# EmbodiedVision/emfusion

Hardware: AMD Instinct MI355X
Metric: frames/sec (integrate+raycast+EM-assoc) (higher is better)
Workload: dtype f32

## Files before the change

emfusion_amd/_lib.py:

```python
from __future__ import annotations

import ctypes as C
import os
import re
from pathlib import Path

PKG_DIR = Path(__file__).resolve().parent
REPO_ROOT = PKG_DIR.parent
LIB_PATH = PKG_DIR / "libemf_hip.so"
HEADER_PATH = REPO_ROOT / "include" / "emf_hip.h"

EMF_OK = 0


class EmfImage(C.Structure):

    _fields_ = [("data", C.c_void_p), ("pitch", C.c_size_t), ("width", C.c_int32),
                ("height", C.c_int32)]


class EmfHipError(RuntimeError):
    def __init__(self, fn: str, code: int, msg: str):
        super().__init__(f"{fn} failed with {code}: {msg}")
        self.code = code
# ... 102 lines not shown
    "emf_hip_trackPrepare": [_FP, _FP, C.c_int, C.c_float, _STREAM],
    "emf_hip_trackIterate": [_FP, _FP, C.c_int, _IMG, C.c_void_p, _FP, C.c_size_t,
                             C.c_int, _STREAM],
    "emf_hip_trackStep": [_FP, _FP, C.c_int, _IMG, C.c_void_p, _FP, C.c_size_t,
                          C.c_int, C.c_int, C.c_void_p, C.c_uint32, C.c_void_p, _STREAM],
    "emf_hip_trackWeightImages": [_FP, _FP, C.c_int, _IMG, C.c_void_p, _FP, C.c_size_t, _FP, _FP, _STREAM],
    "emf_hip_computePoseGradients": [_FP, _FP, _IMG, _F9, _F9, _I3, C.c_float, _FP, _STREAM],
    "emf_hip_integrateBatched": [_FP, _FP, _I3, C.c_int, _FP, _IMG, _IMG, _F9, C.c_int, _FP,
                                 _STREAM],
    "emf_hip_integrateCullScratchBytes": [_I3, C.c_int],
    "emf_hip_integrateBatchedCulled": [_FP, _FP, _I3, C.c_int, _FP, _IMG, _IMG, _F9, _FP, C.c_uint32, _FP, _FP,
                                       _STREAM],
    "emf_hip_integrateDirtyMapBytes": [_I3],
    "emf_hip_integrateBatchedCulledOut": [_FP, _FP, _I3, C.c_int, _FP, _IMG, _IMG, _F9, C.c_void_p, C.c_int, _FP,
                                          C.c_uint32, _FP, _FP, _STREAM],
    "emf_hip_integratePrepareOut": [C.c_void_p, _I3, C.c_int, _FP, _STREAM],
    "emf_hip_visibilityFlags": [_FP, C.c_int, C.c_int, _FP, _FP, _STREAM],
    "emf_hip_resetBrickFlags": [_FP, _I3, _STREAM],
    "emf_hip_packHitKeys": [C.c_int, _I3, _IMG, _IMG, _FP, C.c_int, C.c_int, _STREAM],
    "emf_hip_compositeFromKeys": [_FP, C.c_int, _I3, C.c_int, _I3, _IMG, _IMG, _IMG, _IMG, _IMG,
                                  _IMG, _IMG, _IMG, _IMG, _IMG, _IMG, _IMG, _IMG, C.c_int, _FP,
                                  _STREAM],
    "emf_hip_visibilityFlagsIndexed": [_FP, C.c_int, _I3, C.c_int, _FP, _STREAM],
}


class EmfVolumeOut(C.Structure):
    _fields_ = [("tsdf", C.c_void_p), ("weights", C.c_void_p), ("dirtyPrev", C.c_void_p), ("dirtyNext", C.c_void_p)]


# ... 68 lines not shown
    return _lib


def _bind(lib: C.CDLL) -> C.CDLL:
    for name, argtypes in SIGNATURES.items():
        fn = getattr(lib, name)
        fn.argtypes = argtypes
        fn.restype = C.c_int
    lib.emf_hip_trackScratchBytes.restype = C.c_size_t
    lib.emf_hip_unseenTileBytes.restype = C.c_size_t
    lib.emf_hip_pointStatsScratchBytes.restype = C.c_size_t
    lib.emf_hip_meshScratchBytes.restype = C.c_size_t
    lib.emf_hip_meshScratchBytesBatched.restype = C.c_size_t
    lib.emf_hip_integrateCullScratchBytes.restype = C.c_size_t
    lib.emf_hip_integrateDirtyMapBytes.restype = C.c_size_t
    lib.emf_hip_signMapBytes.restype = C.c_size_t
    lib.emf_hip_raycastFarBoundBytes.restype = C.c_size_t
    lib.emf_hip_relevantTileBytes.restype = C.c_size_t
    lib.emf_hip_peerBufferBytes.restype = C.c_size_t
    lib.emf_hip_peerRaycastSlotBytes.restype = C.c_size_t
    lib.emf_hip_maskAssociationMassBytes.restype = C.c_size_t
    lib.emf_hip_maskAssociationMassScratchBytes.restype = C.c_size_t
    lib.emf_hip_last_error_string.argtypes = []
    lib.emf_hip_last_error_string.restype = C.c_char_p
    return lib


def check(fn_name: str, rc: int) -> None:
    if rc != EMF_OK:
        msg = load().emf_hip_last_error_string().decode(errors="replace")
# ... 2 lines not shown
```

emfusion_amd/csrc/batched.hip:

```cpp
#include <cstdlib>

#include "march_wave.hpp"
#include "peer_core.hpp"

namespace emf_hip {
namespace {

struct PoseTable {
    emf_pose_t p[EMF_MAX_BATCH];
};

__device__ __forceinline__ M33 pose_R(const emf_pose_t& p) {
    return M33{{p.R[0], p.R[1], p.R[2]}, {p.R[3], p.R[4], p.R[5]}, {p.R[6], p.R[7], p.R[8]}};
}
__device__ __forceinline__ V3 pose_t(const emf_pose_t& p) { return V3{p.t[0], p.t[1], p.t[2]}; }


#ifndef EMF_ESTEP_PIXELS
#define EMF_ESTEP_PIXELS 64
#define EMF_ESTEP_LANES 4
#endif
constexpr int kEstepPixels = EMF_ESTEP_PIXELS;
constexpr int kEstepLanes = EMF_ESTEP_LANES;

// ... 720 lines not shown
struct IntegrateOutTable {
    float* tsdf[EMF_MAX_BATCH];
    float* weights[EMF_MAX_BATCH];
    const uint8_t* dirtyPrev[EMF_MAX_BATCH];
    uint8_t* dirtyNext[EMF_MAX_BATCH];
};

struct IntegrateCullArgs {
    IntegrateBatchArgs b;
    int boxStart[EMF_MAX_BATCH + 1];
    unsigned* list;
    unsigned* count;
    IntegrateOutTable out;
    int haveOut;
    int deepTiles;
};


__device__ __forceinline__ IntegrateGeom geom_of(const IntegrateBatchArgs& a, int m) {
    const emf_model_t& md = a.models[m];
    IntegrateGeom g;
    g.depth = a.depth;
    g.invLambda = a.invLambda;
    g.assoc = Img<const float>{md.assoc, static_cast<size_t>(a.w) * sizeof(float)};
    g.w = a.w;
    g.h = a.h;
    g.R = pose_R(a.poses.p[m]);
    g.t = pose_t(a.poses.p[m]);
    g.K = a.K;
    g.pinhole = a.pinhole;
// ... 4 lines not shown
    return g;
}

__global__ __launch_bounds__(256) void k_integrate_cull(const IntegrateCullArgs a) {
    const int i = blockIdx.x * 256 + threadIdx.x;
    {
        float mx = 0.f;
        const int npix = a.b.w * a.b.h, stride = gridDim.x * 256;
        for (int p = i; p < npix; p += stride) {
            const float d = a.b.depth.row(p / a.b.w)[p % a.b.w];
            mx = d > mx ? d : mx;
        }
#pragma unroll
        for (int o = 32; o > 0; o >>= 1) mx = fmaxf(mx, __shfl_xor(mx, o));
        if ((threadIdx.x & 63) == 0 && mx > 0.f) atomicMax(a.count + 1, __float_as_uint(mx));
    }
    bool keep = false;
    unsigned entry = 0;
    if (i < a.boxStart[a.b.nmodels]) {
        int m = 0;
        while (m + 1 < a.b.nmodels && i >= a.boxStart[m + 1]) ++m;
        const bool open = !a.b.visible || a.b.visible[m] != 0;
        if (open || a.haveOut) {
            const IntegrateGeom g = geom_of(a.b, m);
            const int box = i - a.boxStart[m];
            if (open && a.b.stats && box == 0)
                atomicAdd(a.b.stats, static_cast<unsigned long long>(g.n.x) * g.n.y * g.n.z);
            const int nbx = (g.n.x + kBoxX - 1) / kBoxX, nby = (g.n.y + kBoxY - 1) / kBoxY;
            const int bx = box % nbx, by = (box / nbx) % nby, bz = box / (nbx * nby);
            const int x0 = bx * kBoxX, y0 = by * kBoxY, z0 = bz * kBoxZ;
// ... 27 lines not shown
            }
            entry = (static_cast<unsigned>(m) << 24) | static_cast<unsigned>(box);
        }
    }
    const unsigned long long mask = __ballot(keep);
    if (mask == 0ull) return;
    const int lane = threadIdx.x & 63;
    unsigned base = 0;
    if (lane == __ffsll(static_cast<long long>(mask)) - 1) base = atomicAdd(a.count, static_cast<unsigned>(__popcll(mask)));
    base = __shfl(base, __ffsll(static_cast<long long>(mask)) - 1);
    if (keep) a.list[base + __popcll(mask & ((1ull << lane) - 1ull))] = entry;
}

template <bool OUT>
__device__ __forceinline__ void integrate_listed_tile(const IntegrateCullArgs& a, unsigned e, unsigned sub,
                                                      unsigned* lds) {
    const unsigned entry = a.list[e];
    const int m = static_cast<int>(entry >> 24), box = static_cast<int>(entry & 0xffffffu);
    IntegrateGeom g = geom_of(a.b, m);
    g.maxDepthBits = a.deepTiles ? a.count + 1 : nullptr;
    const emf_model_t& md = a.b.models[m];
    const int nbx = (g.n.x + kBoxX - 1) / kBoxX, nby = (g.n.y + kBoxY - 1) / kBoxY;
    const int bx = box % nbx, by = (box / nbx) % nby, bz = box / (nbx * nby);
    const int dx = static_cast<int>(sub % EMF_INT_BOX_X), dy = static_cast<int>((sub / EMF_INT_BOX_X) % EMF_INT_BOX_Y),
              dz = static_cast<int>(sub / (EMF_INT_BOX_X * EMF_INT_BOX_Y));
    const int x0 = (EMF_INT_BOX_X * bx + dx) * kTileX, y0 = (EMF_INT_BOX_Y * by + dy) * kTileY,
              z0 = (EMF_INT_BOX_Z * bz + dz) * kTileZ;
    if (x0 < g.n.x && y0 < g.n.y && z0 < g.n.z) {
        const size_t t = tile_index(g.n, x0, y0, z0), nt = tile_count(g.n);
        uint8_t* sp = md.signMaps ? md.signMaps + t : nullptr;
        if constexpr (OUT) {
            const uint8_t* dp = a.out.dirtyPrev[m];
            const int force = (dp[t] ? 1 : 0) | (dp[nt + t] ? 2 : 0);
            integrate_tile<true>(g, md.tsdf, md.weights, nullptr, x0, y0, z0, lds, a.out.tsdf[m],
                                 a.out.weights[m], force, a.out.dirtyNext[m] + t, a.out.dirtyNext[m] + nt + t,
                                 a.b.visible && a.b.visible[m] == 0, sp, sp ? sp + nt : nullptr,
                                 md.unseenTiles ? md.unseenTiles + t : nullptr);
        } else {
            integrate_tile(g, md.tsdf, md.weights, nullptr, x0, y0, z0, lds, nullptr, nullptr, 0, nullptr, nullptr,
                           false, sp, sp ? sp + nt : nullptr, md.unseenTiles ? md.unseenTiles + t : nullptr);
        }
    }
}

template <bool OUT>
__attribute__((amdgpu_waves_per_eu(EMF_INT_WPE, EMF_INT_WPE)))
__global__ __launch_bounds__(256) void k_integrate_listed(const IntegrateCullArgs a) {
    __shared__ unsigned lds[32];
    const unsigned e = blockIdx.x / kBoxTiles;
    if (e >= *a.count) return;
    integrate_listed_tile<OUT>(a, e, blockIdx.x % kBoxTiles, lds);
}

template <bool OUT>
__global__ __launch_bounds__(256) void k_integrate_listed_rest(const IntegrateCullArgs a, unsigned first) {
    __shared__ unsigned lds[32];
    const unsigned todo = *a.count;
    for (unsigned e = first + blockIdx.x / kBoxTiles; e < todo; e += gridDim.x / kBoxTiles) {
        integrate_listed_tile<OUT>(a, e, blockIdx.x % kBoxTiles, lds);
        __syncthreads();
    }
}

struct DilateBatchArgs {
    const emf_model_t* models;
    int nmodels;
    int brickStart[EMF_MAX_BATCH + 1];
    const int32_t* visible;
};

__global__ __launch_bounds__(256) void k_dilate_batched(const DilateBatchArgs a) {
    const int i = blockIdx.x * 256 + threadIdx.x;
    if (i >= a.brickStart[a.nmodels]) return;
    int m = 0;
// ... 456 lines not shown
    EMF_REQUIRE_PTR(scratch_dev);
    if (nmodels < 1 || nmodels > EMF_MAX_BATCH) return fail(EMF_E_LIMIT, "integratePrepareOut: nmodels = %d", nmodels);
    hipError_t e = hipMemsetAsync(scratch_dev, 0, 2 * sizeof(unsigned), as_stream(stream));
    for (int m = 0; e == hipSuccess && out_host && m < nmodels; ++m) {
        if (!out_host[m].dirtyNext) return fail(EMF_E_NULL, "integratePrepareOut: model %d has no dirtyNext map", m);
        EMF_TRY(check_res(res_host + 3 * m));
        e = hipMemsetAsync(out_host[m].dirtyNext, 0, emf_hip_integrateDirtyMapBytes(res_host + 3 * m), as_stream(stream));
    }
    if (e != hipSuccess) {
        set_error("integratePrepareOut: memset: %s", hipGetErrorString(e));
        return static_cast<int>(e);
    }
    return EMF_OK;
}

int emf_hip_integrateBatchedCulledOut(const emf_model_t* models_dev, const emf_pose_t* poseOC_host,
                                      const int32_t* res_host, int nmodels, const int32_t* visible_dev,
                                      const emf_image_t* depth, const emf_image_t* invLambda,
                                      const float K[9], const emf_volume_out_t* out_host, int prepared,
                                      void* scratch_dev, uint32_t launchBoxes, uint32_t* survivors_out_dev,
                                      uint64_t* stats, emf_stream_t stream) {
    EMF_TRY(check_batch(models_dev, poseOC_host, nmodels, "integrateBatchedCulled"));
    EMF_REQUIRE_PTR(res_host);
    EMF_REQUIRE_PTR(scratch_dev);
    EMF_TRY(check_image(depth, 4, "integrateBatchedCulled: depth"));
    if (invLambda) {
        EMF_TRY(check_image(invLambda, 4, "integrateBatchedCulled: invLambda"));
        EMF_TRY(check_same_size(depth, invLambda, "depth", "invLambda"));
    }
    EMF_REQUIRE_PTR(K);
    IntegrateCullArgs a;
    a.b.models = models_dev;
    a.b.nmodels = nmodels;
    a.boxStart[0] = 0;
    for (int m = 0; m < nmodels; ++m) {
        const int32_t* r = res_host + 3 * m;
// ... 10 lines not shown
    a.b.visible = visible_dev;
    a.b.stats = reinterpret_cast<unsigned long long*>(stats);
    a.b.depth = img<const float>(depth);
    a.b.invLambda = invLambda ? img<const float>(invLambda) : Img<const float>{nullptr, 0};
    a.b.w = depth->width;
    a.b.h = depth->height;
    a.b.K = m33_from(K);
    a.b.pinhole = is_pinhole(a.b.K);
    a.count = static_cast<unsigned*>(scratch_dev);
    a.list = a.count + 4;
    a.out = IntegrateOutTable{};
    a.haveOut = out_host ? 1 : 0;
    const char* dt = std::getenv("EMF_DEEP_TILES");
    const bool deepTiles = !(dt && dt[0] == '0');
    a.deepTiles = deepTiles ? 1 : 0;
    const unsigned total = static_cast<unsigned>(a.boxStart[nmodels]);
    const hipError_t e = prepared ? hipSuccess : hipMemsetAsync(a.count, 0, 2 * sizeof(unsigned), as_stream(stream));
    if (e != hipSuccess) {
        set_error("integrateBatchedCulled: memset: %s", hipGetErrorString(e));
        return static_cast<int>(e);
    }
    if (out_host) {
        for (int m = 0; m < nmodels; ++m) {
            const emf_volume_out_t& o = out_host[m];
            if (!o.tsdf || !o.weights || !o.dirtyPrev || !o.dirtyNext)
                return fail(EMF_E_NULL, "integrateBatchedCulledOut: model %d: tsdf / weights / dirtyPrev / dirtyNext "
                            "of the second copy are all required", m);
            a.out.tsdf[m] = o.tsdf;
            a.out.weights[m] = o.weights;
            a.out.dirtyPrev[m] = o.dirtyPrev;
// ... 45 lines not shown
```

emfusion_amd/csrc/core/EMFusion.cpp:

```cpp
#include "EMFusion.hpp"
#include "EMFusionDetail.hpp"
#include "Readers.hpp"

#include <algorithm>
#include <chrono>
#include <cmath>
#include <cstdio>
#include <cstdlib>
#include <cstring>

namespace emf {

using namespace detail;

EMFusion::EMFusion(const Params& _params, TSDF::Gradients gradients,
                   std::shared_ptr<Communicator> _comm)
    : params(_params),
      gradMode(gradients),
      comm(std::move(_comm)),
      background(_params.globalVolumeDims, _params.globalVoxelSize,
                 _params.globalRelTruncDist * _params.globalVoxelSize, _params.volumePose,
                 _params.tsdfParams, _params.frameSize, gradients),
      depthFiltered(_params.frameSize),
      invLambda(_params.frameSize),
// ... 24 lines not shown
    }
    ignorePerson = params.ignore_person;
    const char* env = std::getenv("EMF_PER_VOLUME");
    forceLegacy = env && env[0] == '1';
    const char* bb = std::getenv("EMF_BG_BANDS");
    bgBands = !(bb && bb[0] == '0');
    const char* ic = std::getenv("EMF_INT_CULL");
    cullBoxes = !(ic && ic[0] == '0');
    const char* oc = debugEnv("EMF_OBJ_CULL");
    objCull = oc && oc[0] == '1';
    if (const char* tc = debugEnv("EMF_TRACK_CHUNK")) trackChunk = std::atoi(tc);
    if (const char* tw = debugEnv("EMF_TRACK_WINDOW")) trackWindow = std::atoi(tw);
    if (const char* fp = debugEnv("EMF_FUSE_POINTS")) fusePoints = fp[0] != '0';
    if (const char* fv = debugEnv("EMF_FUSE_VISIBILITY")) fuseVisibility = fv[0] != '0';
    if (const char* ef = debugEnv("EMF_EARLY_FAR_BOUNDS")) earlyFarBounds = ef[0] != '0';
    const char* bo = std::getenv("EMF_BG_OVERLAP");
    bgOverlap = !(bo && bo[0] == '0');
    const char* fb = std::getenv("EMF_FAR_BOUNDS");
    useFarBounds = !(fb && fb[0] == '0');
    const char* rf = debugEnv("EMF_RAY_FOOTPRINTS");
    useFootprints = !(rf && rf[0] == '0');
    if (const char* mr = std::getenv("EMF_MARCH_ROWS")) {
        marchLanes = std::atoi(mr);
        if (marchLanes != 1 && marchLanes != 2 && marchLanes != 4)
            throw HipError(std::string("EMFusion: EMF_MARCH_ROWS=") + mr + " (1, 2 or 4 lanes per background ray)", EMF_E_ARG);
    }
    const char* au = std::getenv("EMF_ASYNC_UPLOAD");
    asyncUpload = !(au && au[0] == '0');
    const char* lt = std::getenv("EMF_LAMBDA_TABLE");
    useLambdaTable = !(lt && lt[0] == '0');
// ... 191 lines not shown
        tiled &= md.res[0] % 4 == 0;
    }
    integrateCullScratch = DeviceBuffer();
    if (cullBoxes && tiled && TSDF::brickFlagMode() == 0)
        integrateCullScratch = DeviceBuffer(emf_hip_integrateCullScratchBytes(
            resHost.data(), std::min(static_cast<int>(modelsHost.size()), EMF_MAX_BATCH)));
    batched = !forceLegacy && gradMode == TSDF::Gradients::OnTheFly;
    farBounds = DeviceBuffer();
    if (batched && useFarBounds)
        farBounds = DeviceBuffer(2 * emf_hip_raycastFarBoundBytes(static_cast<int>(modelsHost.size()),
                                                                  params.frameSize.width, params.frameSize.height));
    if (batched && !integrateCullScratch.empty() && bgOverlap && bgCullScratch.empty()) {
        background.enableDoubleBuffer();
        bgCullScratch = DeviceBuffer(emf_hip_integrateCullScratchBytes(resHost.data(), 1));
    }
    tableSel = 0;
    hipCheck(hipMemcpy(modelTable.data(), modelsHost.data(),
                       modelsHost.size() * sizeof(emf_model_t), hipMemcpyHostToDevice),
             "model table upload");
    if (batched) {
        if (background.doubleBuffered()) {
            std::vector<emf_model_t> alt = modelsHost;
            const emf_volume_out_t back = background.backBuffers();
            alt[0].tsdf = back.tsdf;
            alt[0].weights = back.weights;
            hipCheck(hipMemcpy(modelTable.as<emf_model_t>() + EMF_MAX_MODELS, alt.data(),
                               alt.size() * sizeof(emf_model_t), hipMemcpyHostToDevice),
                     "model table upload");
        }
        std::vector<int32_t> vis(modelsHost.size(), 0);
// ... 424 lines not shown
void EMFusion::integrateBackgroundAsync() {
    if (!overlapUsable() || bgInFlight) return;
    if (bgBackStale) {
        quiesce();
        background.resyncBack();
        bgBackStale = false;
        bgPrepared = false;
    }
    aux.waitFor(main);
    const emf_pose_t oc = toPose(pose.inv() * background.getPose());
    const double vox = static_cast<double>(resHost[0]) * resHost[1] * resHost[2];
    const emf_image_t il = invLambda.view();
    const emf_volume_out_t out = background.backBuffers();
    {
        auto kt = ktimers.scope(KernelTimers::IntegrateBg, vox, aux);
        emfCheck(emf_hip_integrateBatchedCulledOut(currentTable(), &oc, resHost.data(), 1, nullptr, &depth,
                                                   useLambdaTable ? &il : nullptr, params.intr.val, &out,
                                                   bgPrepared ? 1 : 0, bgCullScratch.data(), 0, nullptr,
                                                   integrateStatsDev.as<uint64_t>(), aux.abi()),
                 "integrateBatchedCulledOut");
    }
    aux.record();
    emf_volume_out_t next = out;
    next.dirtyNext = const_cast<uint8_t*>(out.dirtyPrev);
    emfCheck(emf_hip_integratePrepareOut(&next, resHost.data(), 1, bgCullScratch.data(), aux.abi()),
             "integratePrepareOut");
    bgPrepared = true;
    bgInFlight = true;
    bgListPending = true;
    forkFrame = frameCount;
}

void EMFusion::joinBackground() {
    if (!bgInFlight) return;
    rebuildBackgroundList();
// ... 116 lines not shown
```

emfusion_amd/csrc/core/EMFusion.hpp:

```cpp
#pragma once

#include <algorithm>
#include <list>
#include <map>
#include <string>
#include <memory>
#include <set>
#include <vector>

#include "Communicator.hpp"
#include "KernelTimers.hpp"
#include "ObjTSDF.hpp"
#include "Output.hpp"
#include "TSDF.hpp"

namespace emf {

struct RGBD {
    Size size;
    const float* depth = nullptr;
    const uint8_t* rgb = nullptr;
};

struct FrameInputs {
// ... 320 lines not shown
    DeviceBuffer farBounds;
    int farSel = 0;
    float* farBoundsHalf() const { return farBounds.as<float>() + static_cast<size_t>(farSel) * (farBounds.bytes() / 2 / sizeof(float)); }
    int forkFrame = -2;
    bool farBoundsReady = false;
    bool earlyFarBounds = true;
    bool peerFused = false;
    int bandRowsPending = 0;
    Stream lists{streamPriority("EMF_PRIO_LISTS", -1)};
    bool bgListPending = false;
    bool bgPrepared = false;
    void rebuildBackgroundList();
    void computeFarBounds(const std::vector<emf_pose_t>& co);
    void joinFarBounds();
    DeviceBuffer bgCullScratch;
    bool overlapUsable() const;
    void integrateBackgroundAsync();
    void joinBackground();
    std::vector<emf_model_t> modelsHost;
    std::vector<int32_t> resHost;
    std::vector<float> voxelHost;
    std::vector<uint8_t> scanSlot, listSlot;
    bool anyScan = false;
    DeviceBuffer visibleDev;
    DeviceBuffer integrateStatsDev;
    int32_t* visibleHost = nullptr;
    bool visPending = false;
    std::vector<int32_t> visIds;

    KernelTimers ktimers;
// ... 7 lines not shown
```

emfusion_amd/csrc/device_core.hpp:

```cpp
#pragma once

#include "common.hpp"

namespace emf_hip {

constexpr int kBrick = 4;
constexpr int kBrickShift = 2;
constexpr int kMaxBrickDepth = 3;
enum : uint8_t { kBrickMixed = 0, kBrickAllZero = 1, kBrickAllOne = 2, kBrickAllNegOne = 4 };

__host__ __device__ __forceinline__ int bricks_along(int n) { return (n + kBrick - 1) >> kBrickShift; }

__device__ __forceinline__ unsigned uniform_bits(float v) {
    return (v == 0.f ? kBrickAllZero : 0u) | (v == 1.f ? kBrickAllOne : 0u) |
           (v == -1.f ? kBrickAllNegOne : 0u);
}
__device__ __forceinline__ float brick_constant(uint8_t f) {
    return f == kBrickAllZero ? 0.f : (f == kBrickAllOne ? 1.f : -1.f);
}
__host__ __device__ __forceinline__ size_t brick_count(const I3& n) {
    return static_cast<size_t>(bricks_along(n.x)) * bricks_along(n.y) * bricks_along(n.z);
}
__device__ __forceinline__ uint8_t dilated_flag(const uint8_t* __restrict__ raw, int nbx, int nby,
                                                int nbz, int bx, int by, int bz) {
// ... 27 lines not shown
__device__ __forceinline__ uint8_t flag_class(uint8_t f) { return f & 7u; }
__device__ __forceinline__ int flag_depth(uint8_t f) { return f >> 3; }


struct IntegrateGeom {
    Img<const float> depth, assoc;
    Img<const float> invLambda;
    int w, h;
    M33 R;
    V3 t;
    M33 K;
    I3 n;
    float voxelSize, truncdist, maxWeight;
    bool pinhole;
    const unsigned* maxDepthBits = nullptr;
};

#ifndef EMF_INT_WPE
#define EMF_INT_WPE 5
#endif

inline bool is_pinhole(const M33& K) {
    return K.r0.y == 0.f && K.r1.x == 0.f && K.r2.x == 0.f && K.r2.y == 0.f && K.r2.z == 1.f;
}

enum : int { kSkip = 0, kZeroIfUnseen = 1, kNegIfUnseen = 2, kFuse = 3 };

__device__ __forceinline__ float inv_lambda_at(const M33& K, int px, int py) {
    const float lambda = norm(v3((static_cast<float>(px) - K.r0.z) / K.r0.x,
                                 (static_cast<float>(py) - K.r1.z) / K.r1.y, 1.f));
// ... 204 lines not shown
        f4v t = {v.x, v.y, v.z, v.w};
        __builtin_nontemporal_store(t, reinterpret_cast<f4v*>(p));
    } else {
        *reinterpret_cast<float4*>(p) = v;
    }
}
template <bool NT>
__device__ __forceinline__ float4 load4(const float* p) {
    if (NT && EMF_INT_NT) {
        const f4v t = __builtin_nontemporal_load(reinterpret_cast<const f4v*>(p));
        return make_float4(t.x, t.y, t.z, t.w);
    }
    return *reinterpret_cast<const float4*>(p);
}

template <bool OUT = false>
__device__ __forceinline__ void integrate_tile(const IntegrateGeom& a, float* __restrict__ tsdf,
                                               float* __restrict__ weights,
                                               uint8_t* __restrict__ bricks, int x0, int y0,
                                               int z0, unsigned* lds,
                                               float* __restrict__ tsdfOut = nullptr,
                                               float* __restrict__ weightsOut = nullptr,
                                               int force = 0, uint8_t* dirtyT = nullptr,
                                               uint8_t* dirtyW = nullptr, bool copyOnly = false,
                                               uint8_t* signPos = nullptr, uint8_t* signNeg = nullptr,
                                               uint8_t* unseen = nullptr) {
    const V3 half = half_extent(a.n);
    if ((OUT && copyOnly) || tile_culled(a, half, x0, y0, z0)) {
        if (OUT && force) {
            const int xg = threadIdx.x & 7, yy = (threadIdx.x >> 3) & 7, zs = threadIdx.x >> 6;
            const int x = x0 + 4 * xg, y = y0 + yy;
            if (x < a.n.x && y < a.n.y) {
#pragma unroll
                for (int i = 0; i < 2; ++i) {
                    const int z = z0 + zs + 4 * i;
                    if (z < a.n.z) {
                        const size_t b = (static_cast<size_t>(z) * a.n.y + y) * a.n.x + x;
                        if (force & 1) store4<OUT>(tsdfOut + b, load4<OUT>(tsdf + b));
                        if (force & 2) store4<OUT>(weightsOut + b, load4<OUT>(weights + b));
                    }
                }
            }
        }
        return;
    }
    if (!OUT) {
        tsdfOut = tsdf;
        weightsOut = weights;
    }
    const bool fast = unseen && !bricks && *unseen != 0;
    bool deep = false;
    if (fast && a.maxDepthBits && a.pinhole) {
        float zmin = __builtin_inff();
#pragma unroll
        for (int k = 0; k < 8; ++k)
            zmin = fminf(zmin, voxel_in_camera(a, half, x0 + ((k & 1) ? kTileX - 1 : 0), y0 + ((k & 2) ? kTileY - 1 : 0),
                                               z0 + ((k & 4) ? kTileZ - 1 : 0)).z);
        const float dmax = __uint_as_float(*a.maxDepthBits);
        const float delta = 0.75f / fminf(fabsf(a.K.r0.x), fabsf(a.K.r1.y));
        deep = zmin * (1.f - delta) * (1.f - 1e-5f) - 1e-6f > dmax + a.truncdist * (1.f + 1e-5f);
    }
    const int tid = threadIdx.x;
    const bool haveIl = a.invLambda.data != nullptr;
    bool gotWeight = false;
    int anyChanged = 0;
    bool sawPos = false, sawNeg = false;
    if (bricks) {
        if (tid < 32) lds[tid] = 7u;
        __syncthreads();
    }
    const int xg = tid & 7, yy = (tid >> 3) & 7, zs = tid >> 6;
    const int x = x0 + 4 * xg, y = y0 + yy;
    unsigned bits[2] = {7u, 7u};
    if (x < a.n.x && y < a.n.y) {
        unsigned pix[2][4], inMask = 0, behindMask = 0;
        float n2[2][4];
        bool live[2], touch[2];
        size_t base[2];
#pragma unroll
        for (int i = 0; i < 2; ++i) {
            const int z = z0 + zs + 4 * i;
            live[i] = z < a.n.z;
            const int zc = live[i] ? z : a.n.z - 1;
            base[i] = (static_cast<size_t>(zc) * a.n.y + y) * a.n.x + x;
#pragma unroll
            for (int e = 0; e < 4; ++e) {
                const VoxelShot s = shoot_voxel(a, half, x + e, y, zc);
                pix[i][e] = s.inImage ? (static_cast<unsigned>(s.py) << 16) | static_cast<unsigned>(s.px) : 0u;
                n2[i][e] = s.n2;
                if (s.inImage && live[i]) inMask |= 1u << (4 * i + e);
                if (s.behind && live[i]) behindMask |= 1u << (4 * i + e);
            }
            touch[i] = (((inMask | behindMask) >> (4 * i)) & 15u) != 0;
        }
        float d[2][4], il[2][4];
#pragma unroll
        for (int i = 0; i < 2; ++i)
#pragma unroll
            for (int e = 0; e < 4; ++e) {
// ... 21 lines not shown
#pragma unroll
        for (int i = 0; i < 2; ++i) {
            int changed = 0;
            if (touch[i] && fast) {
                unsigned keep = 0;
#pragma unroll
                for (int e = 0; e < 4; ++e) {
                    VoxelShot s;
                    s.px = pix[i][e] & 0xffffu;
                    s.py = pix[i][e] >> 16;
                    s.inImage = (inMask >> (4 * i + e)) & 1u;
                    s.behind = (behindMask >> (4 * i + e)) & 1u;
                    s.n2 = n2[i][e];
                    float samp = 0.f, aw = 1.f;
                    int kind;
                    if (deep) {
                        kind = s.behind ? kZeroIfUnseen : (!s.inImage ? kSkip : (d[i][e] <= 0.f ? kZeroIfUnseen : kNegIfUnseen));
                    } else {
                        const float ile = haveIl ? il[i][e] : inv_lambda_at(a.K, s.px, s.py);
                        bool band;
                        kind = classify_shot(a, s, d[i][e], ile, samp, band);
                        if (band) aw = a.assoc.row(s.py)[s.px];
                    }
                    if (apply_unseen(kind, samp, aw, a.maxWeight, tv[i][e], wv[i][e])) keep |= 1u << e;
                }
                if (keep) {
                    const float4 tl = load4<OUT>(tsdf + base[i]);
                    if (keep & 1u) tv[i][0] = tl.x;
                    if (keep & 2u) tv[i][1] = tl.y;
                    if (keep & 4u) tv[i][2] = tl.z;
                    if (keep & 8u) tv[i][3] = tl.w;
// ... 386 lines not shown
```

include/emf_hip.h:

```cpp
#ifndef EMF_HIP_H
#define EMF_HIP_H

#include <stddef.h>
#include <stdint.h>

#ifdef __cplusplus
extern "C" {
#endif

#define EMF_HIP_ABI_VERSION 8

typedef struct ihipStream_t* emf_stream_t;

enum {
    EMF_OK = 0,
    EMF_E_NULL = -1,
    EMF_E_SHAPE = -2,
    EMF_E_PITCH = -3,
    EMF_E_ARG = -4,
    EMF_E_LIMIT = -5,
    EMF_E_NODEVICE = -6,
    EMF_E_NOTREADY = -7,
    EMF_E_PEER_TIMEOUT = -8
};
// ... 231 lines not shown
                                   uint32_t* survivors_out_dev, uint64_t* stats, emf_stream_t stream);

typedef struct emf_volume_out {
    float* tsdf;
    float* weights;
    const uint8_t* dirtyPrev;
    uint8_t* dirtyNext;
} emf_volume_out_t;
size_t emf_hip_integrateDirtyMapBytes(const int32_t res[3]);
int emf_hip_integrateBatchedCulledOut(const emf_model_t* models_dev, const emf_pose_t* poseOC_host,
                                      const int32_t* res_host, int nmodels, const int32_t* visible_dev,
                                      const emf_image_t* depth, const emf_image_t* invLambda,
                                      const float K[9], const emf_volume_out_t* out_host, int prepared,
                                      void* scratch_dev, uint32_t launchBoxes, uint32_t* survivors_out_dev,
                                      uint64_t* stats, emf_stream_t stream);
int emf_hip_integratePrepareOut(const emf_volume_out_t* out_host, const int32_t* res_host, int nmodels,
                                void* scratch_dev, emf_stream_t stream);

int emf_hip_visibilityFlags(const int32_t* visCounts, int nmodels, int visibilityThresh,
                            int32_t* visible_dev, int32_t* countsMirror, emf_stream_t stream);

int emf_hip_resetBrickFlags(uint8_t* brickFlags, const int32_t res[3], emf_stream_t stream);


int emf_hip_packHitKeys(int nlocal, const int32_t* listPos_host, const emf_image_t* objRay_host,
                        const emf_image_t* objSeg_host, uint64_t* keys, int width, int height,
                        emf_stream_t stream);

int emf_hip_compositeFromKeys(const uint64_t* keys, int nall, const int32_t* ids_host, int nlocal,
                              const int32_t* listPos_host, const emf_image_t* objRay_host,
// ... 175 lines not shown
```

Before: 1902.

## Certify deep background tiles via per-pixel depth-safe bitmap to skip voxel projection

Adds a bitmap of pixels whose 3x3 depth neighbourhood is all valid, built in the cull kernel. For deep background tiles it uses conservative floating-point error bounds to prove that every voxel projects to a safe pixel, and classifies those voxels from the bitmap held in an LDS window. Only the voxels that cannot be certified are queued and shot individually. This is meant to avoid per-voxel projection and depth loads in deep tiles, at the cost of extra LDS use, more block syncs and a bitmap-building pass over the frame.

```diff
diff --git a/emfusion_amd/_lib.py b/emfusion_amd/_lib.py
--- a/emfusion_amd/_lib.py
+++ b/emfusion_amd/_lib.py
@@ -140,6 +140,9 @@
     "emf_hip_integrateDirtyMapBytes": [_I3],
     "emf_hip_integrateBatchedCulledOut": [_FP, _FP, _I3, C.c_int, _FP, _IMG, _IMG, _F9, C.c_void_p, C.c_int, _FP,
                                           C.c_uint32, _FP, _FP, _STREAM],
+    "emf_hip_depthSafeMapBytes": [C.c_int, C.c_int],
+    "emf_hip_integrateBatchedCulledOutCertified": [_FP, _FP, _I3, C.c_int, _FP, _IMG, _IMG, _F9, C.c_void_p, C.c_int,
+                                                   _FP, C.c_uint32, _FP, _FP, _FP, _STREAM],
     "emf_hip_integratePrepareOut": [C.c_void_p, _I3, C.c_int, _FP, _STREAM],
     "emf_hip_visibilityFlags": [_FP, C.c_int, C.c_int, _FP, _FP, _STREAM],
     "emf_hip_resetBrickFlags": [_FP, _I3, _STREAM],
@@ -238,6 +241,7 @@
     lib.emf_hip_meshScratchBytesBatched.restype = C.c_size_t
     lib.emf_hip_integrateCullScratchBytes.restype = C.c_size_t
     lib.emf_hip_integrateDirtyMapBytes.restype = C.c_size_t
+    lib.emf_hip_depthSafeMapBytes.restype = C.c_size_t
     lib.emf_hip_signMapBytes.restype = C.c_size_t
     lib.emf_hip_raycastFarBoundBytes.restype = C.c_size_t
     lib.emf_hip_relevantTileBytes.restype = C.c_size_t
diff --git a/emfusion_amd/csrc/batched.hip b/emfusion_amd/csrc/batched.hip
--- a/emfusion_amd/csrc/batched.hip
+++ b/emfusion_amd/csrc/batched.hip
@@ -758,6 +758,8 @@
     IntegrateOutTable out;
     int haveOut;
     int deepTiles;
+    unsigned* safeBits;
+    int safeWords;
 };
 
 
@@ -792,6 +794,25 @@
 #pragma unroll
         for (int o = 32; o > 0; o >>= 1) mx = fmaxf(mx, __shfl_xor(mx, o));
         if ((threadIdx.x & 63) == 0 && mx > 0.f) atomicMax(a.count + 1, __float_as_uint(mx));
+    }
+    if (a.safeBits) {
+        const int w = a.b.w, h = a.b.h, nw = a.safeWords * h, lane = threadIdx.x & 63;
+        const int waves = gridDim.x * 4;
+        for (int k = 2 * (i >> 6); k < nw; k += 2 * waves) {
+            const int kw = k + (lane >> 5), y = kw / a.safeWords, x = 32 * (kw - y * a.safeWords) + (lane & 31);
+            bool safe = kw < nw && x >= 1 && x + 1 < w && y >= 1 && y + 1 < h;
+            if (safe) {
+                float d[9];
+#pragma unroll
+                for (int r = 0; r < 3; ++r)
+#pragma unroll
+                    for (int c = 0; c < 3; ++c) d[3 * r + c] = a.b.depth.row(y + r - 1)[x + c - 1];
+#pragma unroll
+                for (int j = 0; j < 9; ++j) safe = safe && d[j] > 0.f;
+            }
+            const unsigned long long m = __ballot(safe);
+            if ((lane & 31) == 0 && kw < nw) a.safeBits[kw] = static_cast<unsigned>(m >> (lane & 32));
+        }
     }
     bool keep = false;
     unsigned entry = 0;
@@ -849,11 +870,13 @@
 
 template <bool OUT>
 __device__ __forceinline__ void integrate_listed_tile(const IntegrateCullArgs& a, unsigned e, unsigned sub,
-                                                      unsigned* lds) {
+                                                      unsigned* lds, CertLds* cert) {
     const unsigned entry = a.list[e];
     const int m = static_cast<int>(entry >> 24), box = static_cast<int>(entry & 0xffffffu);
     IntegrateGeom g = geom_of(a.b, m);
     g.maxDepthBits = a.deepTiles ? a.count + 1 : nullptr;
+    g.safeBits = a.deepTiles ? a.safeBits : nullptr;
+    g.safeWords = a.safeWords;
     const emf_model_t& md = a.b.models[m];
     const int nbx = (g.n.x + kBoxX - 1) / kBoxX, nby = (g.n.y + kBoxY - 1) / kBoxY;
     const int bx = box % nbx, by = (box / nbx) % nby, bz = box / (nbx * nby);
@@ -870,7 +893,7 @@
             integrate_tile<true>(g, md.tsdf, md.weights, nullptr, x0, y0, z0, lds, a.out.tsdf[m],
                                  a.out.weights[m], force, a.out.dirtyNext[m] + t, a.out.dirtyNext[m] + nt + t,
                                  a.b.visible && a.b.visible[m] == 0, sp, sp ? sp + nt : nullptr,
-                                 md.unseenTiles ? md.unseenTiles + t : nullptr);
+                                 md.unseenTiles ? md.unseenTiles + t : nullptr, cert);
         } else {
             integrate_tile(g, md.tsdf, md.weights, nullptr, x0, y0, z0, lds, nullptr, nullptr, 0, nullptr, nullptr,
                            false, sp, sp ? sp + nt : nullptr, md.unseenTiles ? md.unseenTiles + t : nullptr);
@@ -878,21 +901,31 @@
     }
 }
 
+template <bool OUT> struct ListedLds {
+    unsigned flags[32];
+    __device__ CertLds* cert() { return nullptr; }
+};
+template <> struct ListedLds<true> {
+    unsigned flags[32];
+    CertLds certLds;
+    __device__ CertLds* cert() { return &certLds; }
+};
+
 template <bool OUT>
 __attribute__((amdgpu_waves_per_eu(EMF_INT_WPE, EMF_INT_WPE)))
 __global__ __launch_bounds__(256) void k_integrate_listed(const IntegrateCullArgs a) {
-    __shared__ unsigned lds[32];
+    __shared__ ListedLds<OUT> lds;
     const unsigned e = blockIdx.x / kBoxTiles;
     if (e >= *a.count) return;
-    integrate_listed_tile<OUT>(a, e, blockIdx.x % kBoxTiles, lds);
+    integrate_listed_tile<OUT>(a, e, blockIdx.x % kBoxTiles, lds.flags, lds.cert());
 }
 
 template <bool OUT>
 __global__ __launch_bounds__(256) void k_integrate_listed_rest(const IntegrateCullArgs a, unsigned first) {
-    __shared__ unsigned lds[32];
+    __shared__ ListedLds<OUT> lds;
     const unsigned todo = *a.count;
     for (unsigned e = first + blockIdx.x / kBoxTiles; e < todo; e += gridDim.x / kBoxTiles) {
-        integrate_listed_tile<OUT>(a, e, blockIdx.x % kBoxTiles, lds);
+        integrate_listed_tile<OUT>(a, e, blockIdx.x % kBoxTiles, lds.flags, lds.cert());
         __syncthreads();
     }
 }
@@ -1379,12 +1412,28 @@
     return EMF_OK;
 }
 
+size_t emf_hip_depthSafeMapBytes(int width, int height) {
+    if (width < 1 || height < 1) return 0;
+    return static_cast<size_t>((width + 31) / 32) * height * sizeof(unsigned);
+}
+
 int emf_hip_integrateBatchedCulledOut(const emf_model_t* models_dev, const emf_pose_t* poseOC_host,
                                       const int32_t* res_host, int nmodels, const int32_t* visible_dev,
                                       const emf_image_t* depth, const emf_image_t* invLambda,
                                       const float K[9], const emf_volume_out_t* out_host, int prepared,
                                       void* scratch_dev, uint32_t launchBoxes, uint32_t* survivors_out_dev,
                                       uint64_t* stats, emf_stream_t stream) {
+    return emf_hip_integrateBatchedCulledOutCertified(models_dev, poseOC_host, res_host, nmodels, visible_dev, depth,
+                                                      invLambda, K, out_host, prepared, scratch_dev, launchBoxes,
+                                                      survivors_out_dev, stats, nullptr, stream);
+}
+
+int emf_hip_integrateBatchedCulledOutCertified(const emf_model_t* models_dev, const emf_pose_t* poseOC_host,
+                                               const int32_t* res_host, int nmodels, const int32_t* visible_dev,
+                                               const emf_image_t* depth, const emf_image_t* invLambda,
+                                               const float K[9], const emf_volume_out_t* out_host, int prepared,
+                                               void* scratch_dev, uint32_t launchBoxes, uint32_t* survivors_out_dev,
+                                               uint64_t* stats, void* safeMap_dev, emf_stream_t stream) {
     EMF_TRY(check_batch(models_dev, poseOC_host, nmodels, "integrateBatchedCulled"));
     EMF_REQUIRE_PTR(res_host);
     EMF_REQUIRE_PTR(scratch_dev);
@@ -1425,6 +1474,8 @@
     const char* dt = std::getenv("EMF_DEEP_TILES");
     const bool deepTiles = !(dt && dt[0] == '0');
     a.deepTiles = deepTiles ? 1 : 0;
+    a.safeBits = out_host && deepTiles && a.b.pinhole ? static_cast<unsigned*>(safeMap_dev) : nullptr;
+    a.safeWords = (a.b.w + 31) / 32;
     const unsigned total = static_cast<unsigned>(a.boxStart[nmodels]);
     const hipError_t e = prepared ? hipSuccess : hipMemsetAsync(a.count, 0, 2 * sizeof(unsigned), as_stream(stream));
     if (e != hipSuccess) {
diff --git a/emfusion_amd/csrc/core/EMFusion.cpp b/emfusion_amd/csrc/core/EMFusion.cpp
--- a/emfusion_amd/csrc/core/EMFusion.cpp
+++ b/emfusion_amd/csrc/core/EMFusion.cpp
@@ -62,6 +62,7 @@
     if (const char* fp = debugEnv("EMF_FUSE_POINTS")) fusePoints = fp[0] != '0';
     if (const char* fv = debugEnv("EMF_FUSE_VISIBILITY")) fuseVisibility = fv[0] != '0';
     if (const char* ef = debugEnv("EMF_EARLY_FAR_BOUNDS")) earlyFarBounds = ef[0] != '0';
+    if (const char* dc = debugEnv("EMF_DEEP_CERTIFY")) certifyDeep = dc[0] != '0';
     const char* bo = std::getenv("EMF_BG_OVERLAP");
     bgOverlap = !(bo && bo[0] == '0');
     const char* fb = std::getenv("EMF_FAR_BOUNDS");
@@ -283,6 +284,8 @@
         background.enableDoubleBuffer();
         bgCullScratch = DeviceBuffer(emf_hip_integrateCullScratchBytes(resHost.data(), 1));
     }
+    if (!bgCullScratch.empty() && certifyDeep && bgSafeMap.empty())
+        bgSafeMap = DeviceBuffer(emf_hip_depthSafeMapBytes(params.frameSize.width, params.frameSize.height));
     tableSel = 0;
     hipCheck(hipMemcpy(modelTable.data(), modelsHost.data(),
                        modelsHost.size() * sizeof(emf_model_t), hipMemcpyHostToDevice),
@@ -737,11 +740,12 @@
     const emf_volume_out_t out = background.backBuffers();
     {
         auto kt = ktimers.scope(KernelTimers::IntegrateBg, vox, aux);
-        emfCheck(emf_hip_integrateBatchedCulledOut(currentTable(), &oc, resHost.data(), 1, nullptr, &depth,
-                                                   useLambdaTable ? &il : nullptr, params.intr.val, &out,
-                                                   bgPrepared ? 1 : 0, bgCullScratch.data(), 0, nullptr,
-                                                   integrateStatsDev.as<uint64_t>(), aux.abi()),
-                 "integrateBatchedCulledOut");
+        emfCheck(emf_hip_integrateBatchedCulledOutCertified(currentTable(), &oc, resHost.data(), 1, nullptr, &depth,
+                                                            useLambdaTable ? &il : nullptr, params.intr.val, &out,
+                                                            bgPrepared ? 1 : 0, bgCullScratch.data(), 0, nullptr,
+                                                            integrateStatsDev.as<uint64_t>(),
+                                                            bgSafeMap.empty() ? nullptr : bgSafeMap.data(), aux.abi()),
+                 "integrateBatchedCulledOutCertified");
     }
     aux.record();
     emf_volume_out_t next = out;
diff --git a/emfusion_amd/csrc/core/EMFusion.hpp b/emfusion_amd/csrc/core/EMFusion.hpp
--- a/emfusion_amd/csrc/core/EMFusion.hpp
+++ b/emfusion_amd/csrc/core/EMFusion.hpp
@@ -358,6 +358,8 @@
     void computeFarBounds(const std::vector<emf_pose_t>& co);
     void joinFarBounds();
     DeviceBuffer bgCullScratch;
+    DeviceBuffer bgSafeMap;
+    bool certifyDeep = true;
     bool overlapUsable() const;
     void integrateBackgroundAsync();
     void joinBackground();
diff --git a/emfusion_amd/csrc/device_core.hpp b/emfusion_amd/csrc/device_core.hpp
--- a/emfusion_amd/csrc/device_core.hpp
+++ b/emfusion_amd/csrc/device_core.hpp
@@ -65,6 +65,8 @@
     float voxelSize, truncdist, maxWeight;
     bool pinhole;
     const unsigned* maxDepthBits = nullptr;
+    const unsigned* safeBits = nullptr;
+    int safeWords = 0;
 };
 
 #ifndef EMF_INT_WPE
@@ -299,6 +301,169 @@
     return *reinterpret_cast<const float4*>(p);
 }
 
+constexpr int kTileVoxels = kTileX * kTileY * kTileZ;
+constexpr int kCertWindowWords = 384;
+struct CertLds {
+    unsigned win[kCertWindowWords];
+    unsigned count;
+    unsigned short queue[kTileVoxels];
+    unsigned char code[kTileVoxels];
+};
+#ifndef EMF_CERT_LDS
+#define EMF_CERT_LDS 1
+#endif
+
+__device__ __forceinline__ bool certify_deep_tile(const IntegrateGeom& a, const V3& half, int x0, int y0, int z0,
+                                                  bool fast, bool laneValid, const bool live[2], CertLds& L,
+                                                  unsigned& kinds) {
+    const int tid = threadIdx.x;
+    const int x1 = min(x0 + kTileX, a.n.x) - 1, y1 = min(y0 + kTileY, a.n.y) - 1, z1 = min(z0 + kTileZ, a.n.z) - 1;
+    const float s = a.voxelSize;
+    const float fx = a.K.r0.x, cx = a.K.r0.z, fy = a.K.r1.y, cy = a.K.r1.z;
+    float Ax, Ay, Az, Mx, My, zlo, umin, umax, vmin, vmax;
+    {
+        const int k = tid & 7;
+        const int cxi = (k & 1) ? x1 : x0, cyi = (k & 2) ? y1 : y0, czi = (k & 4) ? z1 : z0;
+        const V3 p = voxel_in_camera(a, half, cxi, cyi, czi);
+        const V3 P = project(a, p);
+        const V3 po = v3(fabsf((static_cast<float>(cxi) - half.x) * s), fabsf((static_cast<float>(cyi) - half.y) * s),
+                         fabsf((static_cast<float>(czi) - half.z) * s));
+        const float a0 = fabsf(a.R.r0.x) * po.x + fabsf(a.R.r0.y) * po.y + fabsf(a.R.r0.z) * po.z + fabsf(a.t.x);
+        const float a1 = fabsf(a.R.r1.x) * po.x + fabsf(a.R.r1.y) * po.y + fabsf(a.R.r1.z) * po.z + fabsf(a.t.y);
+        const float a2 = fabsf(a.R.r2.x) * po.x + fabsf(a.R.r2.y) * po.y + fabsf(a.R.r2.z) * po.z + fabsf(a.t.z);
+        Ax = fabsf(fx) * a0 + fabsf(cx) * a2;
+        Ay = fabsf(fy) * a1 + fabsf(cy) * a2;
+        Az = a2;
+        Mx = fabsf(P.x);
+        My = fabsf(P.y);
+        zlo = P.z;
+        umin = umax = P.x / P.z;
+        vmin = vmax = P.y / P.z;
+#pragma unroll
+        for (int o = 1; o < 8; o <<= 1) {
+            Ax = fmaxf(Ax, __shfl_xor(Ax, o));
+            Ay = fmaxf(Ay, __shfl_xor(Ay, o));
+            Az = fmaxf(Az, __shfl_xor(Az, o));
+            Mx = fmaxf(Mx, __shfl_xor(Mx, o));
+            My = fmaxf(My, __shfl_xor(My, o));
+            zlo = fminf(zlo, __shfl_xor(zlo, o));
+            umin = fminf(umin, __shfl_xor(umin, o));
+            umax = fmaxf(umax, __shfl_xor(umax, o));
+            vmin = fminf(vmin, __shfl_xor(vmin, o));
+            vmax = fmaxf(vmax, __shfl_xor(vmax, o));
+        }
+    }
+    const V3 gx = v3(fx * (a.R.r0.x * s) + cx * (a.R.r2.x * s), fy * (a.R.r1.x * s) + cy * (a.R.r2.x * s), a.R.r2.x * s);
+    const V3 gy = v3(fx * (a.R.r0.y * s) + cx * (a.R.r2.y * s), fy * (a.R.r1.y * s) + cy * (a.R.r2.y * s), a.R.r2.y * s);
+    const V3 gz = v3(fx * (a.R.r0.z * s) + cx * (a.R.r2.z * s), fy * (a.R.r1.z * s) + cy * (a.R.r2.z * s), a.R.r2.z * s);
+    const float dxm = static_cast<float>(x1 - x0), dym = static_cast<float>(y1 - y0), dzm = static_cast<float>(z1 - z0);
+    const float as = fabsf(s);
+    const float Sx = (dxm * fabsf(a.R.r0.x) + dym * fabsf(a.R.r0.y) + dzm * fabsf(a.R.r0.z)) * as * fabsf(fx) +
+                     (dxm * fabsf(a.R.r2.x) + dym * fabsf(a.R.r2.y) + dzm * fabsf(a.R.r2.z)) * as * fabsf(cx);
+    const float Sy = (dxm * fabsf(a.R.r1.x) + dym * fabsf(a.R.r1.y) + dzm * fabsf(a.R.r1.z)) * as * fabsf(fy) +
+                     (dxm * fabsf(a.R.r2.x) + dym * fabsf(a.R.r2.y) + dzm * fabsf(a.R.r2.z)) * as * fabsf(cy);
+    const float Sz = (dxm * fabsf(a.R.r2.x) + dym * fabsf(a.R.r2.y) + dzm * fabsf(a.R.r2.z)) * as;
+    const float g = 0x1p-19f, u = 0x1p-24f;
+    const float Dx = g * (3.f * Ax + 2.f * Sx), Dy = g * (3.f * Ay + 2.f * Sy), Dz = g * (3.f * Az + 2.f * Sz);
+    const float zlow = zlo - Dz;
+    const float Qx = (Mx + Dx) / zlow, Qy = (My + Dy) / zlow;
+    const float Ex = 4.f * u * Qx + (Dx + Qx * Dz) / zlow, Ey = 4.f * u * Qy + (Dy + Qy * Dz) / zlow;
+    const float E = fmaxf(Ex, Ey) * (1.f + 0x1p-8f);
+    const bool ok = zlow > 0.f && zlow < 1e30f && E <= 0.25f && Mx + Dx < 1e30f && My + Dy < 1e30f;
+    if (!__syncthreads_and(ok && fast)) return false;
+
+    const float cu0 = fminf(fmaxf(floorf(umin) - 2.f, 0.f), static_cast<float>(a.w - 1)),
+                cu1 = fminf(fmaxf(ceilf(umax) + 2.f, 0.f), static_cast<float>(a.w - 1)),
+                cv0 = fminf(fmaxf(floorf(vmin) - 2.f, 0.f), static_cast<float>(a.h - 1)),
+                cv1 = fminf(fmaxf(ceilf(vmax) + 2.f, 0.f), static_cast<float>(a.h - 1));
+    const int wc0 = static_cast<int>(cu0) >> 5, wy0 = static_cast<int>(cv0);
+    const int nwords = (static_cast<int>(cu1) >> 5) - wc0 + 1, rows = static_cast<int>(cv1) - wy0 + 1;
+    const bool useWin = EMF_CERT_LDS && rows * nwords <= kCertWindowWords;
+    if (useWin)
+        for (int k = tid; k < rows * nwords; k += 256) {
+            const int r = k / nwords;
+            L.win[k] = a.safeBits[static_cast<size_t>(wy0 + r) * a.safeWords + wc0 + (k - r * nwords)];
+        }
+    if (tid == 0) L.count = 0;
+    __syncthreads();
+
+    const int xg = tid & 7, yy = (tid >> 3) & 7, zs = tid >> 6;
+    const int dx = 4 * xg, dy = yy;
+    unsigned pending = 0;
+    kinds = 0;
+    if (laneValid) {
+        int ixs[8], wix[8];
+        unsigned inWin = 0;
+        const V3 Pc = project(a, voxel_in_camera(a, half, x0, y0, z0));
+#pragma unroll
+        for (int i = 0; i < 2; ++i) {
+            const float dz = static_cast<float>(zs + 4 * i);
+            const float bx = fmaf(dz, gz.x, fmaf(static_cast<float>(dy), gy.x, fmaf(static_cast<float>(dx), gx.x, Pc.x)));
+            const float by = fmaf(dz, gz.y, fmaf(static_cast<float>(dy), gy.y, fmaf(static_cast<float>(dx), gx.y, Pc.y)));
+            const float bz = fmaf(dz, gz.z, fmaf(static_cast<float>(dy), gy.z, fmaf(static_cast<float>(dx), gx.z, Pc.z)));
+#pragma unroll
+            for (int e = 0; e < 4; ++e) {
+                const float ef = static_cast<float>(e);
+                const float px = fmaf(ef, gx.x, bx), py = fmaf(ef, gx.y, by), pz = fmaf(ef, gx.z, bz);
+                const float rz = __builtin_amdgcn_rcpf(pz);
+                const int ix = __float2int_rn(px * rz), iy = __float2int_rn(py * rz);
+                const int b = 4 * i + e;
+                ixs[b] = ix;
+                if (useWin) {
+                    const int c = (ix >> 5) - wc0, r = iy - wy0;
+                    const bool in = live[i] && static_cast<unsigned>(c) < static_cast<unsigned>(nwords) &&
+                                    static_cast<unsigned>(r) < static_cast<unsigned>(rows);
+                    wix[b] = in ? r * nwords + c : 0;
+                    inWin |= in ? 1u << b : 0u;
+                } else {
+                    const bool in = live[i] && static_cast<unsigned>(ix) < static_cast<unsigned>(a.w) &&
+                                    static_cast<unsigned>(iy) < static_cast<unsigned>(a.h);
+                    wix[b] = in ? iy * a.safeWords + (ix >> 5) : 0;
+                    inWin |= in ? 1u << b : 0u;
+                }
+            }
+        }
+#pragma unroll
+        for (int b = 0; b < 8; ++b) {
+            const unsigned word = useWin ? L.win[wix[b]] : a.safeBits[wix[b]];
+            if ((inWin >> b) & (word >> (ixs[b] & 31)) & 1u)
+                kinds |= static_cast<unsigned>(kNegIfUnseen) << (2 * b);
+            else if (live[b >> 2])
+                pending |= 1u << b;
+        }
+    }
+    const unsigned np = __popc(pending);
+    unsigned incl = np;
+#pragma unroll
+    for (int o = 1; o < 64; o <<= 1) {
+        const unsigned v = __shfl_up(incl, o);
+        if ((tid & 63) >= o) incl += v;
+    }
+    unsigned base = 0;
+    if ((tid & 63) == 63 && incl) base = atomicAdd(&L.count, incl);
+    base = __shfl(base, 63) + incl - np;
+    for (unsigned m = pending; m; m &= m - 1) {
+        const int b = __ffs(m) - 1, i = b >> 2, e = b & 3;
+        L.queue[base++] = static_cast<unsigned short>((dx + e) | (dy << 5) | ((zs + 4 * i) << 8));
+    }
+    __syncthreads();
+    const unsigned qn = L.count;
+    for (unsigned k = tid; k < qn; k += 256) {
+        const unsigned v = L.queue[k];
+        const VoxelShot sh = shoot_voxel(a, half, x0 + static_cast<int>(v & 31u), y0 + static_cast<int>((v >> 5) & 7u),
+                                         z0 + static_cast<int>(v >> 8));
+        int kind = sh.behind ? kZeroIfUnseen : kSkip;
+        if (sh.inImage) kind = a.depth.row(sh.py)[sh.px] <= 0.f ? kZeroIfUnseen : kNegIfUnseen;
+        L.code[v] = static_cast<unsigned char>(kind);
+    }
+    __syncthreads();
+    for (unsigned m = pending; m; m &= m - 1) {
+        const int b = __ffs(m) - 1, i = b >> 2, e = b & 3;
+        kinds |= static_cast<unsigned>(L.code[(dx + e) | (dy << 5) | ((zs + 4 * i) << 8)]) << (2 * b);
+    }
+    return true;
+}
+
 template <bool OUT = false>
 __device__ __forceinline__ void integrate_tile(const IntegrateGeom& a, float* __restrict__ tsdf,
                                                float* __restrict__ weights,
@@ -309,7 +474,7 @@
                                                int force = 0, uint8_t* dirtyT = nullptr,
                                                uint8_t* dirtyW = nullptr, bool copyOnly = false,
                                                uint8_t* signPos = nullptr, uint8_t* signNeg = nullptr,
-                                               uint8_t* unseen = nullptr) {
+                                               uint8_t* unseen = nullptr, CertLds* certLds = nullptr) {
     const V3 half = half_extent(a.n);
     if ((OUT && copyOnly) || tile_culled(a, half, x0, y0, z0)) {
         if (OUT && force) {
@@ -334,8 +499,8 @@
         weightsOut = weights;
     }
     const bool fast = unseen && !bricks && *unseen != 0;
-    bool deep = false;
-    if (fast && a.maxDepthBits && a.pinhole) {
+    bool geomDeep = false;
+    if (unseen && !bricks && a.maxDepthBits && a.pinhole) {
         float zmin = __builtin_inff();
 #pragma unroll
         for (int k = 0; k < 8; ++k)
@@ -343,9 +508,18 @@
                                                z0 + ((k & 4) ? kTileZ - 1 : 0)).z);
         const float dmax = __uint_as_float(*a.maxDepthBits);
         const float delta = 0.75f / fminf(fabsf(a.K.r0.x), fabsf(a.K.r1.y));
-        deep = zmin * (1.f - delta) * (1.f - 1e-5f) - 1e-6f > dmax + a.truncdist * (1.f + 1e-5f);
-    }
+        geomDeep = zmin * (1.f - delta) * (1.f - 1e-5f) - 1e-6f > dmax + a.truncdist * (1.f + 1e-5f);
+    }
+    const bool deep = fast && geomDeep;
     const int tid = threadIdx.x;
+    const int xg = tid & 7, yy = (tid >> 3) & 7, zs = tid >> 6;
+    const int x = x0 + 4 * xg, y = y0 + yy;
+    unsigned certKinds = 0;
+    bool cert = false;
+    if (OUT && certLds && a.safeBits && geomDeep) {
+        const bool liveZ[2] = {z0 + zs < a.n.z, z0 + zs + 4 < a.n.z};
+        cert = certify_deep_tile(a, half, x0, y0, z0, fast, x < a.n.x && y < a.n.y, liveZ, *certLds, certKinds);
+    }
     const bool haveIl = a.invLambda.data != nullptr;
     bool gotWeight = false;
     int anyChanged = 0;
@@ -354,8 +528,6 @@
         if (tid < 32) lds[tid] = 7u;
         __syncthreads();
     }
-    const int xg = tid & 7, yy = (tid >> 3) & 7, zs = tid >> 6;
-    const int x = x0 + 4 * xg, y = y0 + yy;
     unsigned bits[2] = {7u, 7u};
     if (x < a.n.x && y < a.n.y) {
         unsigned pix[2][4], inMask = 0, behindMask = 0;
@@ -368,6 +540,15 @@
             live[i] = z < a.n.z;
             const int zc = live[i] ? z : a.n.z - 1;
             base[i] = (static_cast<size_t>(zc) * a.n.y + y) * a.n.x + x;
+            if (cert) {
+#pragma unroll
+                for (int e = 0; e < 4; ++e) {
+                    pix[i][e] = 0u;
+                    n2[i][e] = 0.f;
+                }
+                touch[i] = ((certKinds >> (8 * i)) & 0xffu) != 0;
+                continue;
+            }
 #pragma unroll
             for (int e = 0; e < 4; ++e) {
                 const VoxelShot s = shoot_voxel(a, half, x + e, y, zc);
@@ -419,7 +600,9 @@
                     s.n2 = n2[i][e];
                     float samp = 0.f, aw = 1.f;
                     int kind;
-                    if (deep) {
+                    if (cert) {
+                        kind = static_cast<int>((certKinds >> (2 * (4 * i + e))) & 3u);
+                    } else if (deep) {
                         kind = s.behind ? kZeroIfUnseen : (!s.inImage ? kSkip : (d[i][e] <= 0.f ? kZeroIfUnseen : kNegIfUnseen));
                     } else {
                         const float ile = haveIl ? il[i][e] : inv_lambda_at(a.K, s.px, s.py);
diff --git a/include/emf_hip.h b/include/emf_hip.h
--- a/include/emf_hip.h
+++ b/include/emf_hip.h
@@ -269,6 +269,13 @@
                                       const float K[9], const emf_volume_out_t* out_host, int prepared,
                                       void* scratch_dev, uint32_t launchBoxes, uint32_t* survivors_out_dev,
                                       uint64_t* stats, emf_stream_t stream);
+size_t emf_hip_depthSafeMapBytes(int width, int height);
+int emf_hip_integrateBatchedCulledOutCertified(const emf_model_t* models_dev, const emf_pose_t* poseOC_host,
+                                               const int32_t* res_host, int nmodels, const int32_t* visible_dev,
+                                               const emf_image_t* depth, const emf_image_t* invLambda,
+                                               const float K[9], const emf_volume_out_t* out_host, int prepared,
+                                               void* scratch_dev, uint32_t launchBoxes, uint32_t* survivors_out_dev,
+                                               uint64_t* stats, void* safeMap_dev, emf_stream_t stream);
 int emf_hip_integratePrepareOut(const emf_volume_out_t* out_host, const int32_t* res_host, int nmodels,
                                 void* scratch_dev, emf_stream_t stream);
 
```

New measurement: 1723 (median of 2 runs). -9.4%, worse.
